# Bioinfo-Tools/PANGEA-plus

Measured on AMD Instinct MI355X. Metric: classified reads/sec (+ HBM GB/s fraction), 150 bp vs 1 Gbp db, 1/2/4/8 GPU, higher is better.
Workload: dtype u64 (2-bit packed bases, integer scores)

## Files before the change

### pangea-plus_amd/csrc/dust.hip

```cpp
#include <type_traits>

#include "bitops.hpp"
#include "engine.hpp"

namespace pgx {

constexpr int kDustMaxT = 62, kDustLevel = 20;

__device__ __forceinline__ void dust_wave_sync()
{
	asm volatile("s_waitcnt lgkmcnt(0)" ::: "memory");
	__builtin_amdgcn_wave_barrier();
}
struct ScanLane {
	uint32_t w[64];
	uint32_t pad;
};
static_assert(sizeof(ScanLane) / 4 % 2 == 1, "odd word stride");

template <int NR> __device__ __forceinline__ uint64_t reg_window64(const uint64_t (&R)[NR], int pos)
{
	const int wi = __builtin_amdgcn_readfirstlane(pos >> 5), sh = (pos & 31) * 2;
	uint64_t lo = 0, hi = 0;
#pragma unroll
	for (int k = 0; k + 1 < NR; k++)
		if (wi == k) {
			lo = R[k];
			hi = R[k + 1];
		}
	return sh ? (lo >> sh) | (hi << (64 - sh)) : lo;
}

template <int NW>
__global__ __launch_bounds__(64) void k_dust_scan(const uint64_t *__restrict__ fwd, const uint64_t *__restrict__ amb,
						   const uint32_t *__restrict__ len, const uint32_t *__restrict__ woff, uint32_t n,
						   uint32_t *__restrict__ list, uint4 *__restrict__ range, uint32_t *__restrict__ n_list)
{
	constexpr bool REGS = NW > 0;
	constexpr int NR = REGS ? NW + 1 : 1;
	__shared__ ScanLane s_lane[64];
	uint32_t *tab = s_lane[threadIdx.x].w;
	const uint32_t at0 = blockIdx.x * 64u + threadIdx.x;
	const bool has_read = at0 < n;
	const uint32_t r = has_read ? at0 : 0u;
	const int nt = has_read ? (int)len[r] - 2 : 0;
	const uint64_t *rw = fwd + woff[r], *ra = (!REGS && amb) ? amb + woff[r] : nullptr;
	uint64_t R[NR];
	if constexpr (REGS) {
#pragma unroll
		for (int k = 0; k < NR; k++)
			R[k] = k < NW ? rw[k] : 0ull;
	}
	for (int k = 0; k < 64; k++)
		tab[k] = 0u;
	int first = -1, last = -1;
	int p_max = 0, p_last = 0, e0 = -1;
	int size = 0, start = 0, rw_pairs = 0;
	uint64_t in_w = 0, out_w = 0;
	int out_pos = -1;
	int nt_wave = nt;
	if constexpr (REGS) {
		for (int sh = 1; sh < 64; sh <<= 1) {
			const int o = __shfl_xor(nt_wave, sh);
			nt_wave = o > nt_wave ? o : nt_wave;
		}
	}
	for (int b = 0; b < nt_wave; b++) {
		int t = -1;
		if constexpr (REGS) {
			if ((b & 15) == 0)
				in_w = reg_window64(R, b);
			if (b >= kDustMaxT && ((b - kDustMaxT) & 15) == 0)
				out_w = reg_window64(R, b - kDustMaxT);
		}
		if (b < nt) {
			if constexpr (REGS) {
				t = (int)((in_w >> (2 * (b & 15))) & 63ull);
			} else {
				if ((b & 15) == 0)
					in_w = window64(rw, b);
				t = (int)(in_w & 63ull);
				in_w >>= 2;
				if (ra && (window64(ra, b) & 0x15ull))
					t = -1;
				if (t < 0) {
					for (int k = 0; k < 64; k++)
						tab[k] = 0u;
					size = rw_pairs = 0;
					start = b + 1;
				}
			}
		}
		if (t >= 0) {
			uint32_t wt = tab[t];
			int cnt = (int)(wt >> 24);
			if (size >= kDustMaxT) {
				const int ob = b - kDustMaxT;
				int s0;
				if constexpr (REGS) {
					s0 = (int)((out_w >> (2 * (ob & 15))) & 63ull);
				} else {
					if (ob != out_pos || (ob & 15) == 0) {
						out_w = window64(rw, ob);
						out_pos = ob;
					}
					s0 = (int)(out_w & 63ull);
					out_w >>= 2;
					out_pos++;
				}
				if (s0 != t) {
					const uint32_t ws = tab[s0];
					tab[s0] = ws - (1u << 24);
					rw_pairs += cnt - ((int)(ws >> 24) - 1);
					cnt++;
				}
			} else {
				size++;
				rw_pairs += cnt;
				cnt++;
			}
			if (cnt >= 5) {
				const int d = (b - (int)((wt >> 18) & 63u)) & 63;
				const int cand = b - d + 1;
				start = cand > start ? cand : start;
				e0 = e0 < 0 ? b : e0;
			}
			tab[t] = (((wt << 6) | (uint32_t)(b & 63)) & 0xFFFFFFu) | ((uint32_t)cnt << 24);
			int L = b - start + 1;
			L = L < size ? L : size;
			p_max = rw_pairs > p_max ? rw_pairs : p_max;
			if (rw_pairs * 10 > L * kDustLevel) {
				first = first < 0 ? b : first;
				last = b;
				p_last = p_max;
			}
		}
	}
	const unsigned long long listed = __ballot(first >= 0);
	if (listed) {
		uint32_t base = 0;
		const int leader = __ffsll((unsigned long long)listed) - 1;
		if ((int)(threadIdx.x & 63) == leader)
			base = atomicAdd(n_list, (uint32_t)__popcll(listed));
		base = __shfl(base, leader);
		if (first >= 0) {
			const uint32_t at = base + (uint32_t)__popcll(listed & ((1ull << (threadIdx.x & 63)) - 1ull));
			list[at] = r;
			range[at] = make_uint4((uint32_t)first, (uint32_t)last, (uint32_t)p_last, (uint32_t)e0);
		}
	}
}

__device__ __forceinline__ int dust_dpp_up(int v, int last_lane_value)
{
	return __builtin_amdgcn_update_dpp(last_lane_value, v, 0x130, 0xf, 0xf, false);
}

__global__ __launch_bounds__(64) void k_dust_perfect(const uint64_t *__restrict__ fwd, const uint64_t *__restrict__ amb,
						      const uint32_t *__restrict__ len, const uint32_t *__restrict__ woff,
						      const uint32_t *__restrict__ list, const uint4 *__restrict__ range, const uint32_t *__restrict__ n_list,
						      uint64_t *__restrict__ mask, uint8_t *__restrict__ any)
{
	__shared__ uint32_t s_up[3][64];
	const int lane = (int)(threadIdx.x & 63);
	const uint32_t n_in = *n_list;
	if (blockIdx.x >= n_in)
		return;
	uint32_t at = blockIdx.x;
	uint32_t r = list[at];
	uint4 rg = range[at];
	uint32_t L_r = len[r], w_r = woff[r];
	uint32_t r_next = list[at + gridDim.x < n_in ? at + gridDim.x : at];
	for (;;) {
		const uint32_t at_next = at + gridDim.x, at_after = at_next + gridDim.x;
		const bool more = at_next < n_in;
		const uint4 rg_next = range[more ? at_next : at];
		const uint32_t L_next = len[r_next], w_next = woff[r_next];
		const uint32_t r_after = list[at_after < n_in ? at_after : at];
		const int L = (int)L_r, nt = L - 2;
		const uint64_t *rw = fwd + w_r, *ra = amb ? amb + w_r : nullptr;
		uint64_t *mw = mask + w_r;
		const int nw = (L + 63) >> 6;
		for (int w = lane; w < nw; w += 64)
			mw[w] = 0ull;
		const int b_hi = (int)rg.y < nt - 1 ? (int)rg.y : nt - 1;
		const int cap = ((int)rg.z - 1) / 2 + 1 < kDustMaxT ? ((int)rg.z - 1) / 2 + 1 : kDustMaxT;
		const int a_old = (int)rg.x - (kDustMaxT - 1), a_new = (int)rg.w - cap + 1;
		const int a_cut = a_old > a_new ? a_old : a_new;
		const int a_lo = a_cut > 0 ? a_cut : 0;
		const int n_chunks = (b_hi - a_lo + 64) / 64;
		bool marked = false;
		for (int c = n_chunks - 1; c >= 0; c--) {
			const int a0 = a_lo + 64 * c;
			auto triplet = [&](int p) -> int {
				if (p >= nt || (ra && (window64(ra, p) & 0x15ull)))
					return -1;
				return (int)(window64(rw, p) & 63ull);
			};
			const int a = a0 + lane;
			const int ta = triplet(a), t_far = triplet(a + 64);
			const bool has_up = c + 1 < n_chunks;
			const uint32_t upP = has_up ? s_up[0][lane] : 0u, upN = has_up ? s_up[1][lane] : 0u, upQ = has_up ? s_up[2][lane] : 1u;
			dust_wave_sync();
			bool live = a <= b_hi && ta >= 0;
			int tb = ta;
			uint32_t P1 = 0, P2 = 0, Bn = 0, Bq = 1;
			uint32_t myP = 0, myN = 0, myQ = 1;
			int end = -1;
			const int l_max = b_hi - a0 + 1 < cap ? b_hi - a0 + 1 : cap;
			auto steps = [&](auto UP) {
			constexpr bool HAS_UP = decltype(UP)::value;
			int k_zero = 0, k_one = 1, k_none = -1;
			asm volatile("" : "+v"(k_zero), "+v"(k_one), "+v"(k_none));
			for (int l = 2; l <= l_max; l++) {
				const uint32_t nP1 = (uint32_t)dust_dpp_up((int)P1, HAS_UP ? __builtin_amdgcn_readlane((int)upP, l - 1) : k_zero);
				const uint32_t nP2 = (uint32_t)dust_dpp_up((int)P2, HAS_UP && l > 2 ? __builtin_amdgcn_readlane((int)upP, l - 2) : k_zero);
				const uint32_t nBn = (uint32_t)dust_dpp_up((int)Bn, HAS_UP ? __builtin_amdgcn_readlane((int)upN, l - 1) : k_zero);
				const uint32_t nBq = (uint32_t)dust_dpp_up((int)Bq, HAS_UP ? __builtin_amdgcn_readlane((int)upQ, l - 1) : k_one);
				tb = dust_dpp_up(tb, HAS_UP ? __builtin_amdgcn_readlane(t_far, l - 2) : k_none);
				live = live && tb >= 0 && a + l - 1 <= b_hi;
				const uint32_t P = P1 + nP1 - nP2 + (tb == ta ? 1u : 0u);
				const uint32_t q = (uint32_t)(l - 1);
				const bool up_better = __umul24(nBn, Bq) > __umul24(Bn, nBq);
				const uint32_t sn = up_better ? nBn : Bn, sq = up_better ? nBq : Bq;
				const uint32_t lhs = __umul24(sn, q), rhs = __umul24(P, sq);
				if (live && P * 10u > (uint32_t)kDustLevel * q && lhs <= rhs)
					end = a + l + 1;
				const bool sc_better = rhs > lhs;
				P2 = P1;
				P1 = live ? P : 0u;
				Bn = live ? (sc_better ? P : sn) : 0u;
				Bq = live ? (sc_better ? q : sq) : 1u;
				if (c > 0) {
					const uint32_t p0 = (uint32_t)__builtin_amdgcn_readlane((int)P1, 0), n0 = (uint32_t)__builtin_amdgcn_readlane((int)Bn, 0),
						       q0 = (uint32_t)__builtin_amdgcn_readlane((int)Bq, 0);
					const bool me = lane == l;
					myP = me ? p0 : myP;
					myN = me ? n0 : myN;
					myQ = me ? q0 : myQ;
				}
			}
			};
			if (has_up)
				steps(std::true_type{});
			else
				steps(std::false_type{});
			if (c > 0) {
				s_up[0][lane] = myP;
				s_up[1][lane] = myN;
				s_up[2][lane] = myQ;
				dust_wave_sync();
			}
			asm volatile("s_waitcnt vmcnt(0)" ::: "memory");
			if (end >= 0) {
				marked = true;
				for (int k = a; k <= end;) {
					const int w = k >> 6, lo = k & 63;
					const int hi = (end - (w << 6)) < 63 ? end - (w << 6) : 63;
					const uint64_t bits = (hi == 63 ? ~0ull : ((2ull << hi) - 1ull)) & (~0ull << lo);
					atomicOr(reinterpret_cast<unsigned long long *>(mw + w), (unsigned long long)bits);
					k = (w + 1) << 6;
				}
			}
		}
		if (__ballot(marked) && lane == 0)
			any[r] = 1;
		if (!more)
			break;
		at = at_next;
		r = r_next;
		rg = rg_next;
		L_r = L_next;
		w_r = w_next;
		r_next = r_after;
	}
}

__global__ void k_dust_windows(const uint64_t *__restrict__ mask, const uint8_t *__restrict__ any, const uint32_t *__restrict__ len,
			       const uint32_t *__restrict__ woff, const uint32_t *__restrict__ list, const uint32_t *__restrict__ n_list,
			       uint64_t *__restrict__ win_f, uint64_t *__restrict__ win_r)
{
	const uint32_t n_in = *n_list;
	for (uint32_t at = blockIdx.x * blockDim.x + threadIdx.x; at < n_in; at += gridDim.x * blockDim.x) {
		const uint32_t r = list[at];
		if (!any[r])
			continue;
		const int L = (int)len[r];
		const uint32_t w0 = woff[r];
		const int nw = (L + 63) >> 6;
		const int n_valid = L - kWord + 1;
		auto valid_bits = [&](int w) -> uint64_t {
			const int left = n_valid - (w << 6);
			return left <= 0 ? 0ull : (left >= 64 ? ~0ull : ((1ull << left) - 1ull));
		};
		for (int w = 0; w < nw; w++) {
			uint64_t f = valid_bits(w);
			uint64_t lo = mask[w0 + w], hi = w + 1 < nw ? mask[w0 + w + 1] : 0ull;
			auto shr = [](uint64_t &a, uint64_t &b, int k) {
				a |= (a >> k) | (b << (64 - k));
				b |= b >> k;
			};
			shr(lo, hi, 1);
			shr(lo, hi, 2);
			const uint64_t l4 = lo, h4 = hi;
			shr(lo, hi, 4);
			const uint64_t l8 = lo, h8 = hi;
			shr(lo, hi, 8);
			const uint64_t d = lo | ((l8 >> 16) | (h8 << 48)) | ((l4 >> 24) | (h4 << 40));
			f &= ~d;
			win_f[w0 + w] = f;
		}
		for (int w = 0; w < nw; w++) {
			uint64_t rv = valid_bits(w);
			const int s0 = n_valid - (w << 6) - 64;
			uint64_t span;
			if (s0 >= 0) {
				const int wi = s0 >> 6, sh = s0 & 63;
				const uint64_t a = win_f[w0 + wi], b = (sh && wi + 1 < nw) ? win_f[w0 + wi + 1] : 0ull;
				span = sh ? (a >> sh) | (b << (64 - sh)) : a;
			} else if (s0 > -64) {
				span = win_f[w0] << (-s0);
			} else {
				span = 0ull;
			}
			rv = __brevll(span);
			win_r[w0 + w] = rv;
		}
	}
}

static int dust_pass(const pgx_reads *rd, DustBufs &b, hipStream_t stream)
{
	const size_t n = (size_t)rd->n;
	const size_t n_mask = (size_t)rd->n_words + 24;
	PGX_TRY(b.mask.ensure(n_mask));
	PGX_TRY(b.win_f.ensure(n_mask));
	PGX_TRY(b.win_r.ensure(n_mask));
	PGX_TRY(b.any.ensure(n));
	PGX_TRY(b.list.ensure(n));
	PGX_TRY(b.range.ensure(n));
	PGX_TRY(b.n.ensure(2));
	PGX_HIP(hipMemsetAsync(b.any.data(), 0, n, stream));
	PGX_HIP(hipMemsetAsync(b.n.data(), 0, 2 * sizeof(uint32_t), stream));
	const uint64_t *amb = rd->has_amb ? rd->d_fwd_amb.data() : (const uint64_t *)nullptr;
	const dim3 g((unsigned)((n + 63) / 64)), blk(64);
#define PGX_DUST_SCAN(NW)                                                                                                                \
	hipLaunchKernelGGL(k_dust_scan<NW>, g, blk, 0, stream, rd->d_fwd.data(), amb, rd->d_len.data(), rd->d_woff.data(), (uint32_t)n, \
			   b.list.data(), b.range.data(), b.n.data())
	if (amb || rd->max_len > 512)
		PGX_DUST_SCAN(0);
	else if (rd->max_len <= 192)
		PGX_DUST_SCAN(6);
	else if (rd->max_len <= 320)
		PGX_DUST_SCAN(10);
	else
		PGX_DUST_SCAN(16);
#undef PGX_DUST_SCAN
	const unsigned grid2 = (unsigned)std::min<size_t>(n, 256 * 32);
	hipLaunchKernelGGL(k_dust_perfect, dim3(grid2), dim3(64), 0, stream, rd->d_fwd.data(), amb, rd->d_len.data(), rd->d_woff.data(), b.list.data(),
			   b.range.data(), b.n.data(), b.mask.data(), b.any.data());
	hipLaunchKernelGGL(k_dust_windows, dim3((unsigned)std::min<size_t>((n + 127) / 128, 256 * 8)), dim3(128), 0, stream, b.mask.data(), b.any.data(),
			   rd->d_len.data(), rd->d_woff.data(), b.list.data(), b.n.data(), b.win_f.data(), b.win_r.data());
	PGX_HIP(hipGetLastError());
	return 0;
}

int reads_dust(pgx_reads *rd)
{
	const size_t n = (size_t)rd->n;
	rd->has_dust = false;
	if (n == 0)
		return 0;
	DustBufs &b = rd->dustb;
	PGX_TRY(dust_pass(rd, b, 0));
	std::vector<uint8_t> &h_any = rd->h_read_dust;
	h_any.resize(n);
	PGX_TRY(b.any.download(h_any.data(), n));
	bool some = false;
	for (size_t i = 0; i < n && !some; i++)
		some = h_any[i] != 0;
	if (!some) {
		h_any.clear();
		return 0;
	}
	rd->has_dust = true;
	return 0;
}

int reads_dust_again(const pgx_reads *rd, DustBufs &b, hipStream_t stream)
{
	if (rd->n == 0)
		return 0;
	return dust_pass(rd, b, stream);
}

int dust_read_back(const char *who, const pgx_reads *rd, const DustBufs &b, hipStream_t stream, uint8_t *any_out, uint32_t *woff_out,
		   uint64_t *mask_out, uint64_t *win_f_out, uint64_t *win_r_out, int64_t cap_words, int64_t *n_words_out)
{
	const size_t n = (size_t)rd->n, nw = (size_t)rd->n_words;
	if (n_words_out)
		*n_words_out = (int64_t)nw;
	if (woff_out)
		std::copy(rd->h_woff.begin(), rd->h_woff.begin() + (ptrdiff_t)std::min(n + 1, rd->h_woff.size()), woff_out);
	if (!any_out && !mask_out && !win_f_out && !win_r_out)
		return 0;
	if ((mask_out || win_f_out || win_r_out) && cap_words < (int64_t)nw)
		return fail(PGX_E_ARG, "%s: the word arrays hold %lld words, the batch has %lld", who, (long long)cap_words, (long long)nw);
	if (n == 0)
		return 0;
	if (b.any.n < n || b.mask.n < nw || b.win_f.n < nw || b.win_r.n < nw)
		return fail(PGX_E_ARG, "%s: no DUST pass over a batch of this size has run into these buffers", who);
	PGX_HIP(hipStreamSynchronize(stream));
	if (any_out)
		PGX_TRY(b.any.download(any_out, n));
	if (mask_out)
		PGX_TRY(b.mask.download(mask_out, nw));
	if (win_f_out)
		PGX_TRY(b.win_f.download(win_f_out, nw));
	if (win_r_out)
		PGX_TRY(b.win_r.download(win_r_out, nw));
	return 0;
}

}

extern "C" int pgx_reads_get_dust(const pgx_reads *r, uint8_t *any_out, uint32_t *woff_out, uint64_t *mask_out, uint64_t *win_f_out,
				  uint64_t *win_r_out, int64_t cap_words, int64_t *n_words_out)
{
	if (!r)
		return pgx::fail(PGX_E_ARG, "pgx_reads_get_dust: null argument");
	return pgx::dust_read_back("pgx_reads_get_dust", r, r->dustb, 0, any_out, woff_out, mask_out, win_f_out, win_r_out, cap_words, n_words_out);
}

extern "C" int pgx_reads_redo_dust(pgx_reads *r)
{
	if (!r)
		return pgx::fail(PGX_E_ARG, "pgx_reads_redo_dust: null argument");
	if (int rc = pgx::require_device())
		return rc;
	return pgx::guard("pgx_reads_redo_dust", [&]() -> int {
		const bool had = r->has_dust;
		if (int rc = pgx::reads_dust(r))
			return rc;
		if (r->has_dust != had)
			return pgx::fail(PGX_E_NODEVICE, "pgx_reads_redo_dust: the masks of the batch changed between two passes");
		return 0;
	});
}
```

Baseline: 125.2 million.

## Restructure register-path DUST scan around LDS atomics and a deferred update pipeline

The register-resident DUST scan becomes its own function. Bases are held as 32-bit words that shift down every 16 bases, and each triplet-table update is done with LDS fetch_add, fetch_sub and fetch_xor atomics that pack count and last-position fields. The bookkeeping for base b is deferred until step b+1 so atomic latency overlaps the next step, and the window-start/size tracking is simplified into a single L counter with min logic. This targets the per-base read-modify-write dependency chain and the dynamic register window selection. It adds subtle changes to the semantics (the cnt>=4 test on pre-increment values, the L bookkeeping, and e0 defaulting to INT_MAX when no hit occurs) that may alter outputs.

```diff
diff --git a/pangea-plus_amd/csrc/dust.hip b/pangea-plus_amd/csrc/dust.hip
--- a/pangea-plus_amd/csrc/dust.hip
+++ b/pangea-plus_amd/csrc/dust.hip
@@ -18,17 +18,152 @@
 };
 static_assert(sizeof(ScanLane) / 4 % 2 == 1, "odd word stride");
 
-template <int NR> __device__ __forceinline__ uint64_t reg_window64(const uint64_t (&R)[NR], int pos)
-{
-	const int wi = __builtin_amdgcn_readfirstlane(pos >> 5), sh = (pos & 31) * 2;
-	uint64_t lo = 0, hi = 0;
+constexpr uint32_t kScanLeave = 1u << 24, kScanEnter = (1u << 24) + (1u << 30);
+static_assert(kDustLevel % 10 == 0, "the test 10 r_w > level * L as r_w > (level / 10) * L");
+
+template <int NW>
+__device__ __forceinline__ void dust_scan_regs(uint32_t *tab, const uint64_t *rw, int nt, int &first, int &last, int &p_last, int &e0)
+{
+	constexpr int ND = 2 * NW + 6;
+	uint32_t D[ND];
 #pragma unroll
-	for (int k = 0; k + 1 < NR; k++)
-		if (wi == k) {
-			lo = R[k];
-			hi = R[k + 1];
-		}
-	return sh ? (lo >> sh) | (hi << (64 - sh)) : lo;
+	for (int k = 0; k < NW; k++) {
+		const uint2 w = reinterpret_cast<const uint2 *>(rw)[k];
+		D[4 + 2 * k] = w.x;
+		D[5 + 2 * k] = w.y;
+	}
+	D[0] = D[1] = D[2] = D[3] = D[ND - 2] = D[ND - 1] = 0u;
+	int nt_wave = nt;
+	for (int sh = 1; sh < 64; sh <<= 1) {
+		const int o = __shfl_xor(nt_wave, sh);
+		nt_wave = o > nt_wave ? o : nt_wave;
+	}
+	nt_wave = __builtin_amdgcn_readfirstlane(nt_wave);
+	int L = -1, rw_pairs = 0, p_max = 0, e0_min = 0x7fffffff;
+	uint32_t old_s = kScanLeave, old_t = 0u, *at_t = tab + 64;
+	auto finish = [&](int b) __attribute__((always_inline)) {
+		const int cnt = (int)__builtin_amdgcn_ubfe(old_t, 24, 6);
+		const int cs = (int)__builtin_amdgcn_ubfe(old_s, 24, 6);
+		rw_pairs += cnt - cs + 1;
+		const uint32_t sh = (old_t >> 30) * 6u;
+		const uint32_t o = (old_t >> sh) & 63u;
+		__hip_atomic_fetch_xor(at_t, (o ^ (uint32_t)(b & 63)) << sh, __ATOMIC_RELAXED, __HIP_MEMORY_SCOPE_WORKGROUP);
+		const bool five = cnt >= 4;
+		const int d = (b - (int)o) & 63;
+		L = min(L + 1, five ? d : kDustMaxT);
+		e0_min = min(e0_min, five ? b : 0x7fffffff);
+		p_max = max(p_max, rw_pairs);
+		if (rw_pairs > L * (kDustLevel / 10)) {
+			asm volatile("");
+			const bool mine = b < nt;
+			first = mine && first < 0 ? b : first;
+			last = mine ? b : last;
+			p_last = mine ? p_max : p_last;
+		}
+	};
+	auto step = [&](int b, int k, bool full) __attribute__((always_inline)) {
+		uint32_t ns = kScanLeave;
+		if (full) {
+			uint32_t s0 = k + 2 < 14 ? __builtin_amdgcn_ubfe(D[0], 2 * (k + 2), 6) : (uint32_t)((((uint64_t)D[0] | ((uint64_t)D[1] << 32)) >> (2 * k + 4)) & 63ull);
+			asm("" : "+v"(s0));
+			ns = __hip_atomic_fetch_sub(tab + s0, kScanLeave, __ATOMIC_RELAXED, __HIP_MEMORY_SCOPE_WORKGROUP);
+		}
+		uint32_t t = k < 14 ? __builtin_amdgcn_ubfe(D[4], 2 * k, 6) : (uint32_t)((((uint64_t)D[4] | ((uint64_t)D[5] << 32)) >> (2 * k)) & 63ull);
+		asm("" : "+v"(t));
+		uint32_t *at = tab + t;
+		const uint32_t nv = __hip_atomic_fetch_add(at, kScanEnter, __ATOMIC_RELAXED, __HIP_MEMORY_SCOPE_WORKGROUP);
+		__builtin_amdgcn_sched_barrier(0);
+		finish(b - 1);
+		old_s = ns;
+		old_t = nv;
+		at_t = at;
+	};
+	auto move_down = [&]() __attribute__((always_inline)) {
+#pragma unroll
+		for (int i = 0; i + 1 < ND; i++)
+			D[i] = D[i + 1];
+	};
+	int b0 = 0;
+	for (; b0 + 16 <= nt_wave; b0 += 16) {
+		if (b0 < 48) {
+#pragma unroll
+			for (int k = 0; k < 16; k++)
+				step(b0 + k, k, false);
+		} else if (b0 == 48) {
+#pragma unroll
+			for (int k = 0; k < 16; k++)
+				step(48 + k, k, 48 + k >= kDustMaxT);
+		} else {
+#pragma unroll
+			for (int k = 0; k < 16; k++)
+				step(b0 + k, k, true);
+		}
+		move_down();
+	}
+	for (int b = b0; b < nt_wave; b++)
+		step(b, b - b0, b >= kDustMaxT);
+	finish(nt_wave - 1);
+	e0 = e0_min;
+}
+
+__device__ __forceinline__ void dust_scan_mem(uint32_t *tab, const uint64_t *rw, const uint64_t *ra, int nt, int &first, int &last, int &p_last, int &e0)
+{
+	int p_max = 0;
+	int size = 0, start = 0, rw_pairs = 0;
+	uint64_t in_w = 0, out_w = 0;
+	int out_pos = -1;
+	for (int b = 0; b < nt; b++) {
+		if ((b & 15) == 0)
+			in_w = window64(rw, b);
+		int t = (int)(in_w & 63ull);
+		in_w >>= 2;
+		if (ra && (window64(ra, b) & 0x15ull))
+			t = -1;
+		if (t < 0) {
+			for (int k = 0; k < 64; k++)
+				tab[k] = 0u;
+			size = rw_pairs = 0;
+			start = b + 1;
+			continue;
+		}
+		uint32_t wt = tab[t];
+		int cnt = (int)(wt >> 24);
+		if (size >= kDustMaxT) {
+			const int ob = b - kDustMaxT;
+			if (ob != out_pos || (ob & 15) == 0) {
+				out_w = window64(rw, ob);
+				out_pos = ob;
+			}
+			const int s0 = (int)(out_w & 63ull);
+			out_w >>= 2;
+			out_pos++;
+			if (s0 != t) {
+				const uint32_t ws = tab[s0];
+				tab[s0] = ws - (1u << 24);
+				rw_pairs += cnt - ((int)(ws >> 24) - 1);
+				cnt++;
+			}
+		} else {
+			size++;
+			rw_pairs += cnt;
+			cnt++;
+		}
+		if (cnt >= 5) {
+			const int d = (b - (int)((wt >> 18) & 63u)) & 63;
+			const int cand = b - d + 1;
+			start = cand > start ? cand : start;
+			e0 = e0 < 0 ? b : e0;
+		}
+		tab[t] = (((wt << 6) | (uint32_t)(b & 63)) & 0xFFFFFFu) | ((uint32_t)cnt << 24);
+		int L = b - start + 1;
+		L = L < size ? L : size;
+		p_max = rw_pairs > p_max ? rw_pairs : p_max;
+		if (rw_pairs * 10 > L * kDustLevel) {
+			first = first < 0 ? b : first;
+			last = b;
+			p_last = p_max;
+		}
+	}
 }
 
 template <int NW>
@@ -36,106 +171,20 @@
 						   const uint32_t *__restrict__ len, const uint32_t *__restrict__ woff, uint32_t n,
 						   uint32_t *__restrict__ list, uint4 *__restrict__ range, uint32_t *__restrict__ n_list)
 {
-	constexpr bool REGS = NW > 0;
-	constexpr int NR = REGS ? NW + 1 : 1;
 	__shared__ ScanLane s_lane[64];
 	uint32_t *tab = s_lane[threadIdx.x].w;
 	const uint32_t at0 = blockIdx.x * 64u + threadIdx.x;
 	const bool has_read = at0 < n;
 	const uint32_t r = has_read ? at0 : 0u;
 	const int nt = has_read ? (int)len[r] - 2 : 0;
-	const uint64_t *rw = fwd + woff[r], *ra = (!REGS && amb) ? amb + woff[r] : nullptr;
-	uint64_t R[NR];
-	if constexpr (REGS) {
-#pragma unroll
-		for (int k = 0; k < NR; k++)
-			R[k] = k < NW ? rw[k] : 0ull;
-	}
+	const uint64_t *rw = fwd + woff[r];
 	for (int k = 0; k < 64; k++)
 		tab[k] = 0u;
-	int first = -1, last = -1;
-	int p_max = 0, p_last = 0, e0 = -1;
-	int size = 0, start = 0, rw_pairs = 0;
-	uint64_t in_w = 0, out_w = 0;
-	int out_pos = -1;
-	int nt_wave = nt;
-	if constexpr (REGS) {
-		for (int sh = 1; sh < 64; sh <<= 1) {
-			const int o = __shfl_xor(nt_wave, sh);
-			nt_wave = o > nt_wave ? o : nt_wave;
-		}
-	}
-	for (int b = 0; b < nt_wave; b++) {
-		int t = -1;
-		if constexpr (REGS) {
-			if ((b & 15) == 0)
-				in_w = reg_window64(R, b);
-			if (b >= kDustMaxT && ((b - kDustMaxT) & 15) == 0)
-				out_w = reg_window64(R, b - kDustMaxT);
-		}
-		if (b < nt) {
-			if constexpr (REGS) {
-				t = (int)((in_w >> (2 * (b & 15))) & 63ull);
-			} else {
-				if ((b & 15) == 0)
-					in_w = window64(rw, b);
-				t = (int)(in_w & 63ull);
-				in_w >>= 2;
-				if (ra && (window64(ra, b) & 0x15ull))
-					t = -1;
-				if (t < 0) {
-					for (int k = 0; k < 64; k++)
-						tab[k] = 0u;
-					size = rw_pairs = 0;
-					start = b + 1;
-				}
-			}
-		}
-		if (t >= 0) {
-			uint32_t wt = tab[t];
-			int cnt = (int)(wt >> 24);
-			if (size >= kDustMaxT) {
-				const int ob = b - kDustMaxT;
-				int s0;
-				if constexpr (REGS) {
-					s0 = (int)((out_w >> (2 * (ob & 15))) & 63ull);
-				} else {
-					if (ob != out_pos || (ob & 15) == 0) {
-						out_w = window64(rw, ob);
-						out_pos = ob;
-					}
-					s0 = (int)(out_w & 63ull);
-					out_w >>= 2;
-					out_pos++;
-				}
-				if (s0 != t) {
-					const uint32_t ws = tab[s0];
-					tab[s0] = ws - (1u << 24);
-					rw_pairs += cnt - ((int)(ws >> 24) - 1);
-					cnt++;
-				}
-			} else {
-				size++;
-				rw_pairs += cnt;
-				cnt++;
-			}
-			if (cnt >= 5) {
-				const int d = (b - (int)((wt >> 18) & 63u)) & 63;
-				const int cand = b - d + 1;
-				start = cand > start ? cand : start;
-				e0 = e0 < 0 ? b : e0;
-			}
-			tab[t] = (((wt << 6) | (uint32_t)(b & 63)) & 0xFFFFFFu) | ((uint32_t)cnt << 24);
-			int L = b - start + 1;
-			L = L < size ? L : size;
-			p_max = rw_pairs > p_max ? rw_pairs : p_max;
-			if (rw_pairs * 10 > L * kDustLevel) {
-				first = first < 0 ? b : first;
-				last = b;
-				p_last = p_max;
-			}
-		}
-	}
+	int first = -1, last = -1, p_last = 0, e0 = -1;
+	if constexpr (NW > 0)
+		dust_scan_regs<NW>(tab, rw, nt, first, last, p_last, e0);
+	else
+		dust_scan_mem(tab, rw, amb ? amb + woff[r] : nullptr, nt, first, last, p_last, e0);
 	const unsigned long long listed = __ballot(first >= 0);
 	if (listed) {
 		uint32_t base = 0;
```

Result: faster. 126.9 million, median of 6 (+1.4%).
